# albertfgu/diffwave-sashimi

Measured on AMD Instinct MI355X. Metric: audio samples/sec (generate.py-style reverse-diffusion sampling, T=200), higher is better.
Workload: dtype f32-equivalent (3-term bf16 split, 6 products, fp32 accumulate); 1 GPU; wnet_h256_d36_T200; backbone=wavenet, batch_per_gpu=16, L=16000, T=200, parallelism=independent clips per GPU, no collective, sampler=hipGraph replay, on-device Philox noise

## Files before the change

### diffwave-sashimi_amd/csrc/common.hip

```cpp
#include "dws_common.h"
#include "model.h"

#include <mutex>

namespace dws {

static thread_local char g_err[1024] = "";

int set_error(int code, const char* fmt, ...) {
    va_list ap;
    va_start(ap, fmt);
    vsnprintf(g_err, sizeof(g_err), fmt, ap);
    va_end(ap);
    return code;
}

static std::mutex g_prof_mu;
static bool g_prof_on = false;
static std::string g_prof_substr;
static std::vector<std::pair<hipEvent_t, hipEvent_t>> g_prof_events;

bool profile_active() { return g_prof_on; }

ProfileScope::ProfileScope(const char* name, hipStream_t s) : on(false), stream(s), e0(nullptr), e1(nullptr) {
    if (!g_prof_on) return;
    if (strstr(name, g_prof_substr.c_str()) == nullptr) return;
    hipStreamCaptureStatus st = hipStreamCaptureStatusNone;
    if (hipStreamIsCapturing(s, &st) != hipSuccess || st != hipStreamCaptureStatusNone) return;
    if (hipEventCreate(&e0) != hipSuccess || hipEventCreate(&e1) != hipSuccess) return;
    on = true;
    hipEventRecord(e0, stream);
}

ProfileScope::~ProfileScope() {
    if (!on) return;
    hipEventRecord(e1, stream);
    std::lock_guard<std::mutex> lk(g_prof_mu);
    g_prof_events.emplace_back(e0, e1);
}

__global__ void multi_copy_kernel(const CopyJob* __restrict__ jobs, int parts) {
    const CopyJob j = jobs[blockIdx.x];
    for (int64_t i = (int64_t)blockIdx.y * blockDim.x + threadIdx.x; i < j.n; i += (int64_t)parts * blockDim.x) j.dst[i] = j.src[i];
}

int launch_multi_copy(const CopyJob* table_dev, int njobs, hipStream_t s) {
    const int parts = 8;
    hipLaunchKernelGGL(multi_copy_kernel, dim3((unsigned)njobs, parts), dim3(256), 0, s, table_dev, parts);
    DWS_HIP(hipGetLastError());
    return DWS_OK;
}

}
// ... 63 lines not shown
```

### diffwave-sashimi_amd/csrc/dws_common.h

```cpp
#pragma once
#include <hip/hip_runtime.h>
#include <cstdarg>
#include <cstdint>
#include <cstdio>
#include <cstring>
#include <map>
#include <string>
#include <vector>

#include "../../include/dws.h"

namespace dws {

int set_error(int code, const char* fmt, ...);

#define DWS_CHECK(cond, code, ...)                         \
    do {                                                   \
        if (!(cond)) return ::dws::set_error((code), __VA_ARGS__); \
    } while (0)

#define DWS_HIP(expr)                                                                   \
    do {                                                                                \
        hipError_t _e = (expr);                                                         \
        if (_e != hipSuccess)                                                           \
// ... 47 lines not shown
    return fmaf(-w, (p * t) * ez, fmaxf(x, 0.f));
}
__device__ __forceinline__ float dws_gelu_grad(float x) {
    float ez;
    const float cdf = dws_norm_cdf(x, ez);
    return fmaf(x * 0.39894228040143267794f, ez, cdf);
}

constexpr int DWS_MAX_DEVICES = 16;
inline int current_device_slot() {
    int d = 0;
    (void)hipGetDevice(&d);
    return ((unsigned)d < (unsigned)DWS_MAX_DEVICES) ? d : 0;
}

__device__ __forceinline__ int xcd_remap(int bid, int nwg) {
    const int NX = 8;
    int xcd = bid % NX, idx = bid / NX;
    int q = nwg / NX, r = nwg % NX;
    int base = (xcd < r) ? xcd * (q + 1) : r * (q + 1) + (xcd - r) * q;
    return base + idx;
}

}
```

### diffwave-sashimi_amd/csrc/fftconv_kernels.hip

```cpp
#include <cstdio>
#include <cstdlib>
#include <type_traits>
#include <vector>

#include "fftconv.h"

#include "fft_core.h"

namespace dws {

__device__ __forceinline__ float gelu_f(float x) { return dws_gelu(x); }
__device__ __forceinline__ int brev(int k, int bits) { return brev_bits(k, bits); }

struct NoStamp {
    __device__ __forceinline__ void operator()() const {}
    __device__ __forceinline__ void loads_landed() const {}
};
constexpr int FFT_TRACE_SLOTS = 16, FFT_TRACE_ROWS = 4;
struct WaveStamp {
    unsigned long long* slot;
    int k;
    bool lane0;
    __device__ __forceinline__ void operator()() {
        const unsigned long long t = __builtin_amdgcn_s_memtime();
// ... 669 lines not shown
    static constexpr int THREADS = M / 16;
    static constexpr size_t LDS = (size_t)(M + M / 16) * 8;
    static constexpr bool FUSED = FftPlan<LOG2M>::TAIL4 && !FftPlan<LOG2M>::ODD;
};

bool fftconv_supported(int L, int* log2m) {
    if (L < 16 || (L & 1)) return false;
    int lg = 4;
    while ((1 << lg) < L) ++lg;
    if (lg < 10) lg = 10;
    if (lg > 14) return false;
    if (log2m) *log2m = lg;
    return true;
}

static int cu_count() {
    static int n_dev[DWS_MAX_DEVICES] = {};
    int& n = n_dev[current_device_slot()];
    if (!n) {
        int dev = 0;
        hipDeviceProp_t prop;
        if (hipGetDevice(&dev) == hipSuccess && hipGetDeviceProperties(&prop, dev) == hipSuccess) n = prop.multiProcessorCount;
        if (n <= 0) n = 256;
    }
    return n;
}

template <int LOG2M>
static int fft_trace_launch(FftConvArgs a, int nwg, hipStream_t s) {
    using C = FcCfg<LOG2M>;
    static const char* names[12] = {"", "loads landed", "top pass", "fwd P1", "fwd P2", "fwd tail", "pointwise", "inv tail",
                                    "inv P2", "inv P1", "bottom + stores", "closing barrier"};
    static const bool fused = C::FUSED && getenv("DWS_FFT_NO_FUSED_TAIL") == nullptr;
    auto kern = fused ? fftconv_kernel<LOG2M, C::THREADS, true, C::FUSED> : fftconv_kernel<LOG2M, C::THREADS, true>;
    constexpr int NP = FftPlan<LOG2M>::N16 - 1;
    const int T4 = (FftPlan<LOG2M>::TAIL4 && !fused) ? 1 : 0, NST = 3 + NP + T4 + 1 + T4 + NP + 2;
    static bool attr_dev[DWS_MAX_DEVICES] = {};
    bool& attr = attr_dev[current_device_slot()];
    if (!attr) {
        DWS_HIP(hipFuncSetAttribute((const void*)kern, hipFuncAttributeMaxDynamicSharedMemorySize, (int)C::LDS));
        attr = true;
    }
// ... 223 lines not shown
```

### diffwave-sashimi_amd/csrc/wavenet.h

```cpp
#pragma once
#include "dws_common.h"

namespace dws {

constexpr int WN_LAYER_KC = 32;
constexpr int WN_BX3_KC = 16;

struct WnLayerArgs {
    const float* x_in;
    float* x_out;
    float* skip;
    const float* part_t;
    int part_t_bstride;
    const float* A1;
    const float* A2;
    const float* Abt;
    int abt_bstride;
    const int* step_idx;
    int abt_tstride, part_t_tstride;
    const float* Wd;
    const float* Wr;
    const float* Ws;
    const float* bias1;
    const float* bias2;
    const float* melc;
    int mel_bstride;
    float* gate_ws;
    float* hsave;
    int B, L, dilation, first_layer, last_layer;
    const float* wscale;
    unsigned long long* trace;
};

struct WnFinalArgs {
    const float* skip;
    const float* Af;
    const float* Wf;
    const float* bf;
    const float* Wz;
    const float* bz;
    float* out;
    float* tap;
    float scale;
    int B, L, Cout;
    int af_scaled;
// ... 17 lines not shown
int launch_wn_layer_generic(int C, int S, const WnLayerArgs& a, hipStream_t s);
bool wn_final_mfma_supported(int S);
bool wn_layer_wino_supported(int C, int S);
int launch_wino_dconv(const float* w, float* out, int C, hipStream_t s);
int launch_wn_wino_bias(const float* Wd_all, const float* part_t, float* Abt, int NL, int B, int C, hipStream_t s);
int launch_wn_layer_wino(int C, int S, const WnLayerArgs& a, hipStream_t s);
bool wn_layer_bf16x3_supported(int C, int S);
int launch_wn_layer_bf16x3(int C, int S, const WnLayerArgs& a, hipStream_t s);
int launch_pack_a_bf16x3(const float* w, void* out, int M, int K, hipStream_t s);
int launch_wn_bias_tap_bf16(const float* Wd_all, const float* part_t, const float* bias1_all, void* Abt, int NL, int B, int C,
                            hipStream_t s);
enum { WN_SPLIT_BF16X6 = 0, WN_SPLIT_F16X3 = 1 };
inline int wn_split_terms(int split) { return split == WN_SPLIT_F16X3 ? 2 : 3; }
bool wn_layer_bx6_supported(int C, int S);
int launch_wn_layer_bx6(int C, int S, const WnLayerArgs& a, int split, hipStream_t s);
int launch_weight_scale(const float* w, size_t n, const float* bias, int nb, const float* bias_b, int nb_b, float* out, hipStream_t s);
int launch_pack_a1_bx6(const float* w, void* out, int C, int split, const float* scale, hipStream_t s);
int launch_pack_a_bx6(const float* w, void* out, int M, int K, int split, const float* scale, hipStream_t s);
int launch_gemm_bx6(const float* A, const float* B, float* C, int M, int N, int K, int split, float sa, float sb, hipStream_t s);
int launch_wn_final(int S, const WnFinalArgs& a, hipStream_t s);

}
```

### diffwave-sashimi_amd/csrc/wavenet_bx6.hip

```cpp
#include <cstdlib>
#include <type_traits>

#include "bf16_split.h"
#include "wavenet.h"
#include "wn_trace.h"

namespace dws {

#ifndef BX6_PF3
#define BX6_PF3 1
#endif
#ifndef BX6_PF2
#define BX6_PF2 2
#endif
#define BX6_PF(NT) ((NT) == 2 ? BX6_PF2 : BX6_PF3)
#ifndef BX6_T_SLOTS
#define BX6_T_SLOTS 0, 2, 3, 4, 6, 7, 9
#endif

typedef float bx6_f32x4 __attribute__((ext_vector_type(4)));

#ifdef BX6_ABL_NO_NT
#define BX6_NT 0
#else
#define BX6_NT 2
#endif
__device__ __forceinline__ bx6_f32x4 bx6_load_f4(__amdgpu_buffer_rsrc_t r, int voff, int soff) {
    return __builtin_bit_cast(bx6_f32x4, __builtin_amdgcn_raw_buffer_load_b128(r, voff, soff, BX6_NT));
}
__device__ __forceinline__ void bx6_store_f4(bx6_f32x4 v, __amdgpu_buffer_rsrc_t r, int voff, int soff) {
    typedef unsigned int u4 __attribute__((ext_vector_type(4)));
    __builtin_amdgcn_raw_buffer_store_b128(__builtin_bit_cast(u4, v), r, voff, soff, BX6_NT);
// ... 112 lines not shown
    static constexpr int RAW_FLOATS = KC * 4 * NP;
    static constexpr int BOP_BYTES = (KC / 8) * 4 * NT * NP * 16;
    static constexpr int STAGE_FLOATS = 2 * RAW_FLOATS + 2 * BOP_BYTES / 4;
    static constexpr int GATE_BYTES = (C / 8) * NT * 64 * 16;
    static constexpr int MAIN_FLOATS = STAGE_FLOATS > GATE_BYTES / 4 ? STAGE_FLOATS : GATE_BYTES / 4;
    static constexpr int TR_FLOATS = 32 * 64;
    static constexpr int LDS_FLOATS = MAIN_FLOATS + WAVES * TR_FLOATS;
    static constexpr int TITEMS = (KC / 4) * NP * 2;
    static constexpr bool HALVES = WAVES == 8 && NT == 3;
    static constexpr int SW = HALVES ? WAVES / 2 : WAVES;
    static constexpr int NPIECE = KC / (2 * SW);
    static_assert(C % 32 == 0 && S % C == 0 && C % KC == 0 && KC % 16 == 0 && KC % (2 * SW) == 0 && (SW & (SW - 1)) == 0 &&
                  (!HALVES || NCB % 2 == 0) && (TITEMS % NTH == 0) && LDS_FLOATS * 4 <= 163840, "channel counts");
};

template <typename P, int C, int S, bool EXTRA>
__global__ __launch_bounds__(C * 2, (C >= 128 ? 2 : 1)) void wn_layer_bx6_kernel(WnLayerArgs a, int log2d) {
    using T = Bx6Tile<C, S, P::NT>;
    using v8 = typename P::v8;
    using v4 = typename P::v4;
    constexpr int NT = P::NT, NPR = P::NP, NA = 2 * P::NT;
    constexpr int KC = T::KC, MS = T::MS, WAVES = T::WAVES, NCB = T::NCB, NTH = T::NTH, NKB = T::NKB;
    __shared__ __attribute__((aligned(16))) float lds[T::LDS_FLOATS];
    float* const Xraw = lds;
    char* const Bop = reinterpret_cast<char*>(lds + 2 * T::RAW_FLOATS);
    char* const gt = reinterpret_cast<char*>(lds);

    const int tid = threadIdx.x;
    const int lane = tid & 63;
    const int wave = __builtin_amdgcn_readfirstlane(tid >> 6);
    const int l31 = lane & 31, lhi = lane >> 5;
    const int L = a.L, dil = 1 << log2d;
    float* const trw = lds + T::MAIN_FLOATS + wave * T::TR_FLOATS;

    const int nblk = (L + 2 * dil - 1) >> (log2d + 1);
    const int ntl = ((nblk << log2d) + 31) >> 5;
    const int tile = xcd_remap(blockIdx.x, gridDim.x);
    const int b = __builtin_amdgcn_readfirstlane(tile / ntl);
    const int tic = tile % ntl;
#ifdef WN_TILE_ORDER_LINEAR
    const int q0 = __builtin_amdgcn_readfirstlane(tic * 32);
#else
    const int q0 = __builtin_amdgcn_readfirstlane(log2d >= 6 ? ((tic % nblk) << log2d) + (tic / nblk) * 32 : tic * 32);
#endif
    const int q = q0 + l31;
    const int p = ((q >> log2d) << (log2d + 1)) + (q & (dil - 1));

    const float* __restrict__ xb = a.x_in + (size_t)b * C * L;
    unsigned long long* __restrict__ trc = a.trace ? a.trace + ((size_t)blockIdx.x * WAVES + wave) * 32 : nullptr;
    auto stamp = [&](int i) {
        if (trc) {
            const unsigned long long t = __builtin_amdgcn_s_memtime();
            if (lane == 0) trc[i] = t;
        }
    };
    stamp(0);

    const int mt1[2] = {wave, C / 32 + wave};
    int mt2[1 + MS];
    mt2[0] = wave;
#pragma unroll
    for (int m = 0; m < MS; ++m) mt2[1 + m] = C / 32 + wave * MS + m;
    float av1[2][4], ab1[2], av2[1 + MS];
    {
        const float* Abt = a.Abt + (size_t)b * a.abt_bstride + step_row_off(a.step_idx, a.abt_tstride);
#pragma unroll
        for (int m = 0; m < 2; ++m) {
            const int row = mt1[m] * 32 + l31;
#pragma unroll
            for (int j = 0; j < 4; ++j) av1[m][j] = Abt[j * 2 * C + row];
            ab1[m] = a.bias1[row];
        }
#pragma unroll
        for (int m = 0; m < 1 + MS; ++m) av2[m] = a.bias2[mt2[m] * 32 + l31];
    }
    const float ws1 = P::SCALED ? a.wscale[0] : 1.f, ws2 = P::SCALED ? a.wscale[1] : 1.f;
    const float inv1 = 1.f / (ws1 * P::SX), inv2 = 1.f / (ws2 * P::SG);

    const bool al16 = (L % 4 == 0) && ((((size_t)a.x_in | (size_t)a.x_out | (size_t)a.skip) & 15) == 0);
    const bool contig = al16 && log2d <= 4;
    const bool x4 = contig || (al16 && log2d >= 2);
    __amdgpu_buffer_rsrc_t rXall = __builtin_amdgcn_make_buffer_rsrc((void*)xb, 0, C * L * 4, 0x00020000);
    const int pbase = (q0 >> log2d) << (log2d + 1);
    const int ob = contig ? 32 + (p - pbase) - dil : l31;
    const int os = contig ? dil : 32;
    const int x0l = p - pbase, x1l = x0l + dil;
    const int gcol0 = contig ? x0l : l31, gcol1 = contig ? x1l : 32 + l31;
    int voffA, voffB;
    if (contig) {
        const int pp = pbase - 32 + 4 * (lane & 31);
        voffA = ((unsigned)pp < (unsigned)L) ? (lhi * L + pp) * 4 : 0x7ffffff0;
        voffB = 0;
    } else if (x4) {
        const int s4 = (lane >> 3) & 3, qq = q0 + 4 * (lane & 7);
        const int pp = ((qq >> log2d) << (log2d + 1)) + (qq & (dil - 1)) + (s4 - 1) * dil;
        voffA = ((unsigned)pp < (unsigned)L) ? (lhi * L + pp) * 4 : 0x7ffffff0;
        voffB = 0;
    } else {
        voffA = (p + (lhi - 1) * dil) * 4;
        voffB = (p + (lhi + 1) * dil) * 4;
    }
#ifdef BX6_ABL_NO_ROT
// ... 28 lines not shown
    auto stage_dma = [&](int cbi) {
#pragma unroll
        for (int i = 0; i < NPIECE; ++i) stage_piece(cbi, i);
    };

    constexpr int TK = T::TITEMS / NTH, T_UNITS = 7;
    struct TState {
        float d[TK][2][3];
        v4 pa[TK][NT], pb[TK][NT];
    };
    auto transform_unit = [&](int c1, int u, TState& ts) __attribute__((always_inline)) {
        const float* xs = Xraw + (c1 & 1) * T::RAW_FLOATS;
        char* bo = Bop + (c1 & 1) * T::BOP_BYTES;
#pragma unroll
        for (int k = 0; k < TK; ++k) {
            const int i = tid + NTH * k;
            const int gi = __builtin_amdgcn_readfirstlane(i >> 6);
            const int g4 = (gi * 2 + lhi) % (KC / 4);
            const int jp = __builtin_amdgcn_readfirstlane((gi * 2) / (KC / 4));
            const bool p1 = jp != 0;
            const int h = u / 3, w = u % 3;
            if (u == T_UNITS - 1) {
                char* dst = bo + ((((g4 >> 1) * 4 + 2 * jp) * NT) * 32 + l31) * 16 + (g4 & 1) * 8;
#pragma unroll
                for (int t = 0; t < NT; ++t) {
                    *reinterpret_cast<v4*>(dst + t * 512) = ts.pa[k][t];
                    *reinterpret_cast<v4*>(dst + (NT + t) * 512) = ts.pb[k][t];
                }
            } else if (w == 0) {
                const int oa = p1 ? 3 * os : 0;
#pragma unroll
                for (int e = 0; e < 2; ++e) {
// ... 172 lines not shown
        if (cb + 2 < NCB && stages(cb + 2)) stage_dma(cb + 2);
#endif
        if (cb + 1 < NCB) do_step(cb, std::integral_constant<int, 0>{}, std::true_type{});
        else do_step(cb, std::integral_constant<int, 0>{}, std::false_type{});
        do_steps_from1(cb);
        stamp(8 + 2 * cb);
#ifndef BX6_ABL_NO_DMA_WAIT
        __builtin_amdgcn_s_waitcnt(0x0F70 | NAF);
#endif
#ifndef BX6_ABL_NO_BARRIER
        __syncthreads();
#endif
        stamp(9 + 2 * cb);
    }
    stamp(2);

    const int L4 = L * 4;
    const bool first = a.first_layer, last = a.last_layer;
    __amdgpu_buffer_rsrc_t rXo = __builtin_amdgcn_make_buffer_rsrc((void*)(a.x_out + (size_t)b * C * L), 0, C * L * 4, 0x00020000);
    __amdgpu_buffer_rsrc_t rSk = __builtin_amdgcn_make_buffer_rsrc((void*)(a.skip + (size_t)b * S * L), 0, S * L * 4, 0x00020000);
    const int p0 = ((q0 >> log2d) << (log2d + 1)) + (q0 & (dil - 1));
    int voff4;
    {
        const int n4 = (lane & 15) >> 3;
        const int pos4 = (contig ? pbase + 32 * n4 : p0 + n4 * dil) + 4 * (lane & 7);
        voff4 = (pos4 < L) ? ((lane >> 4) * L + pos4) * 4 : 0x7ffffff0;
    }
    constexpr bool PRELOAD = MS == 1;
    const int voff4s = first ? 0x7ffffff0 : voff4;
    auto load_pre = [&](int m, bx6_f32x4 (&dst)[8]) {
#pragma unroll
        for (int i = 0; i < 8; ++i) {
            if (m == 0) dst[i] = *reinterpret_cast<const bx6_f32x4*>(trw + ((lane >> 4) + 4 * i) * 64 + 4 * (lane & 15));
            else dst[i] = bx6_load_f4(rSk, voff4s, ((wave * MS + (m - 1)) * 32 + 4 * i) * L4);
        }
    };
    bx6_f32x4 pre[PRELOAD ? 1 + MS : 1][8];
    if (PRELOAD && al16) {
#pragma unroll
        for (int m = 1; m < 1 + MS; ++m) load_pre(m, pre[PRELOAD ? m : 0]);
    }

    const float* melb = (EXTRA && a.melc) ? a.melc + (size_t)(a.mel_bstride ? b : 0) * 2 * C * L : nullptr;
#pragma unroll
    for (int qd = 0; qd < 4; ++qd) {
        float g0[4], g1[4];
#pragma unroll
        for (int e = 0; e < 4; ++e) {
            const int r = qd * 4 + e;
            const int ch = wave * 32 + e + 8 * qd + 4 * lhi;
#pragma unroll
            for (int n = 0; n < 2; ++n) {
                const int pos = p + n * dil;
                float ht, hs;
                if (n == 0) {
                    ht = (acc[0][0][r] + acc[0][1][r]) + acc[0][2][r];
                    hs = (acc[1][0][r] + acc[1][1][r]) + acc[1][2][r];
                } else {
                    ht = (acc[0][1][r] - acc[0][2][r]) - acc[0][3][r];
                    hs = (acc[1][1][r] - acc[1][2][r]) - acc[1][3][r];
                }
                if (P::SCALED) { ht *= inv1; hs *= inv1; }
                if (EXTRA && melb && pos < L) {
                    ht += melb[(size_t)ch * L + pos];
                    hs += melb[(size_t)(C + ch) * L + pos];
                }
                if (EXTRA && a.hsave && pos < L) {
                    float* __restrict__ hb = a.hsave + (size_t)b * 2 * C * L;
                    hb[(size_t)ch * L + pos] = ht;
                    hb[(size_t)(C + ch) * L + pos] = hs;
                }
                const float g = bx6_gate(ht, hs) * P::SG;
                if (n == 0) g0[e] = g; else g1[e] = g;
            }
        }
        v4 s0[NT], s1[NT];
        P::split4(g0, s0);
        P::split4(g1, s1);
        char* dst = gt + ((wave * 4 + qd) * NT * 64) * 16 + lhi * 8;
#pragma unroll
        for (int t = 0; t < NT; ++t) {
            *reinterpret_cast<v4*>(dst + (t * 64 + gcol0) * 16) = s0[t];
            *reinterpret_cast<v4*>(dst + (t * 64 + gcol1) * 16) = s1[t];
        }
    }
    stamp(3);

    __amdgpu_buffer_rsrc_t rA2 = __builtin_amdgcn_make_buffer_rsrc((void*)a.A2, 0, (C + S) * C * 2 * NT, 0x00020000);
    v8 c_cur[1 + MS][NT], c_nxt[1 + MS][NT];
    auto load_a2 = [&](v8 (&dst)[1 + MS][NT], int kb, int m0) {
#pragma unroll
        for (int m = m0; m < 1 + MS; ++m)
#pragma unroll
            for (int t = 0; t < NT; ++t)
                dst[m][t] = __builtin_bit_cast(v8, __builtin_amdgcn_raw_buffer_load_b128(rA2, lane16, ((mt2[m] * NKB + kb) * NT + t) * 1024, 0));
    };
    const int rot2 = rot * (KC / 16);
    auto kblock_of = [&](int kb) { const int k = kb + rot2; return k >= NKB ? k - NKB : k; };
    bx_f32x16 acc2[1 + MS][2];
    auto gemm2 = [&](auto WITH_RES) {
        constexpr int M0 = decltype(WITH_RES)::value ? 0 : 1;
        load_a2(c_cur, kblock_of(0), M0);
        {
            const v8 bf = P::bvals(lhi ? 0.f : P::SG, 0.f);
            bx_f32x16 zero;
#pragma unroll
            for (int r = 0; r < 16; ++r) zero[r] = 0.f;
#pragma unroll
            for (int m = M0; m < 1 + MS; ++m) {
                v8 af[NT];
                P::rank2(av2[m] * ws2, 0.f, lhi == 0, af);
#pragma unroll
                for (int n = 0; n < 2; ++n) {
                    acc2[m][n] = zero;
#pragma unroll
                    for (int t = NT - 1; t >= 0; --t) acc2[m][n] = P::mfma(af[t], bf, acc2[m][n]);
                }
            }
        }
        __syncthreads();
        stamp(4);
        const char* gb = gt + lhi * (NT * 64 * 16) + l31 * 16;
#pragma unroll 2
        for (int kb = 0; kb < NKB; ++kb) {
            const int kbn = (kb + 1 < NKB) ? kb + 1 : kb;
            load_a2(c_nxt, kblock_of(kbn), M0);
            __builtin_amdgcn_sched_barrier(0);
            const char* gk = gb + kblock_of(kb) * (2 * NT * 64 * 16);
            v8 bq[2][NT];
#pragma unroll
            for (int n = 0; n < 2; ++n)
#pragma unroll
                for (int t = 0; t < NT; ++t) bq[n][t] = *reinterpret_cast<const v8*>(gk + (t * 64 + n * 32) * 16);
#pragma unroll
            for (int t = 0; t < NPR; ++t)
#pragma unroll
                for (int m = M0; m < 1 + MS; ++m)
// ... 8 lines not shown
    };
    if (last) gemm2(std::false_type{});
    else gemm2(std::true_type{});
    stamp(5);

    const float rs = 0.70710678118654752440f;
    if (al16) {
#pragma unroll
        for (int m = 0; m < 1 + MS; ++m) {
            if (m == 0 && last) continue;
            if (!PRELOAD || m == 0) load_pre(m, pre[0]);
            asm volatile("s_waitcnt lgkmcnt(0)" ::: "memory");
#pragma unroll
            for (int n = 0; n < 2; ++n)
#pragma unroll
                for (int r = 0; r < 16; ++r) trw[((r & 3) + 8 * (r >> 2) + 4 * lhi) * 64 + n * 32 + l31] = P::SCALED ? acc2[m][n][r] * inv2 : acc2[m][n][r];
            asm volatile("s_waitcnt lgkmcnt(0)" ::: "memory");
            const int row0 = (m == 0) ? wave * 32 : (wave * MS + (m - 1)) * 32;
#pragma unroll
            for (int i = 0; i < 8; ++i) {
                const bx6_f32x4 v = *reinterpret_cast<const bx6_f32x4*>(trw + ((lane >> 4) + 4 * i) * 64 + 4 * (lane & 15));
                bx6_f32x4 o = pre[PRELOAD ? m : 0][i] + v;
                if (m == 0) o = o * rs;
                bx6_store_f4(o, m == 0 ? rXo : rSk, voff4, (row0 + 4 * i) * L4);
                asm volatile("s_nop 1" ::: "memory");
            }
            asm volatile("" ::: "memory");
        }
    } else {
        int voffn[2];
#pragma unroll
        for (int n = 0; n < 2; ++n) {
            const int pos = contig ? pbase + 32 * n + l31 : p + n * dil;
            voffn[n] = (pos < L) ? (4 * lhi * L + pos) * 4 : 0x7ffffff0;
        }
#pragma unroll
        for (int n = 0; n < 2; ++n) {
            if (!last) {
                const int s0 = (wave * 32) * L4;
#pragma unroll
                for (int r = 0; r < 16; ++r) {
                    const int so = s0 + ((r & 3) + 8 * (r >> 2)) * L4;
                    const float x = __builtin_bit_cast(float, __builtin_amdgcn_raw_buffer_load_b32(rXall, voffn[n], so, 0));
                    const float v = (x + (P::SCALED ? acc2[0][n][r] * inv2 : acc2[0][n][r])) * rs;
                    __builtin_amdgcn_raw_buffer_store_b32(__builtin_bit_cast(unsigned, v), rXo, voffn[n], so, 0);
                }
            }
#pragma unroll
            for (int m = 0; m < MS; ++m) {
                const int s0 = ((wave * MS + m) * 32) * L4;
#pragma unroll
                for (int r = 0; r < 16; ++r) {
                    const int so = s0 + ((r & 3) + 8 * (r >> 2)) * L4;
                    const float old = first ? 0.f : __builtin_bit_cast(float, __builtin_amdgcn_raw_buffer_load_b32(rSk, voffn[n], so, 0));
                    const float v = old + (P::SCALED ? acc2[1 + m][n][r] * inv2 : acc2[1 + m][n][r]);
                    __builtin_amdgcn_raw_buffer_store_b32(__builtin_bit_cast(unsigned, v), rSk, voffn[n], so, 0);
                }
            }
        }
    }
    stamp(6);
    if (trc) {
        __builtin_amdgcn_s_waitcnt(0);
        stamp(7);
    }
}

template <typename P, int C, int S>
static int launch_bx6_t(const WnLayerArgs& a, int log2d, hipStream_t s) {
    ProfileScope ps(P::NT == 3 ? "wn_layer_bx6" : "wn_layer_f16x3", s);
    using T = Bx6Tile<C, S, P::NT>;
    const int dil = 1 << log2d;
    const int nblk = (a.L + 2 * dil - 1) / (2 * dil);
    const int ntl = (nblk * dil + 31) / 32;
    const int ntiles = a.B * ntl;
    static const bool trace = std::getenv("DWS_BX6_TRACE") != nullptr;
    if (trace && !a.melc && !a.hsave) {
        wino_trace_launch(ntiles, T::WAVES, a, s, [&](const WnLayerArgs& at) {
            hipLaunchKernelGGL((wn_layer_bx6_kernel<P, C, S, false>), dim3(ntiles), dim3(T::NTH), 0, s, at, log2d);
        }, P::NT == 3 ? "bx6" : "f16x3");
        return DWS_OK;
    }
    if (a.melc || a.hsave) hipLaunchKernelGGL((wn_layer_bx6_kernel<P, C, S, true>), dim3(ntiles), dim3(T::NTH), 0, s, a, log2d);
    else hipLaunchKernelGGL((wn_layer_bx6_kernel<P, C, S, false>), dim3(ntiles), dim3(T::NTH), 0, s, a, log2d);
    return DWS_OK;
}

bool wn_layer_bx6_supported(int C, int S) {
    return (C == 64 && S == 64) || (C == 128 && S == 128) || (C == 128 && S == 256) || (C == 256 && S == 256);
}

template <typename P>
static int launch_bx6_p(int C, int S, const WnLayerArgs& a, int log2d, hipStream_t s) {
    if (C == 64 && S == 64) return launch_bx6_t<P, 64, 64>(a, log2d, s);
    if (C == 128 && S == 128) return launch_bx6_t<P, 128, 128>(a, log2d, s);
    if (C == 128 && S == 256) return launch_bx6_t<P, 128, 256>(a, log2d, s);
    if (C == 256 && S == 256) return launch_bx6_t<P, 256, 256>(a, log2d, s);
    return set_error(DWS_ERR_UNSUPPORTED, "wn_layer_bx6: (C=%d,S=%d) not instantiated", C, S);
}

// ... 70 lines not shown
```

### diffwave-sashimi_amd/csrc/wavenet_model.hip

```cpp
#include <cmath>

#include "conditioner.h"
#include "model.h"
#include "wavenet.h"
#include "wavenet_backward.h"

namespace dws {

struct WaveNetModel : dws_model {
    int Cin, Cout, C, S, NL, cycle, Ein, Emid, Eout, MB;
    bool cond, mfma_layer, mfma_final;
    bool bf16x3 = false;
    bool bf16x6 = false;
    bool f16x3 = false;
    DevBuf wscale;
    bool wino_opt = true;
    bool wino_fits(int64_t nL) const {
        return (int64_t)std::max(C, S) * nL * 4 < ((int64_t)1 << 31) && nL + 4 * ((int64_t)1 << (cycle - 1)) < ((int64_t)1 << 28);
    }
    bool wino() const { return wino_opt && mfma_layer && !bf16x3 && !bf16x6 && !f16x3 && wn_layer_wino_supported(C, S) && (L == 0 || wino_fits(L)); }
    bool wino_rows() const { return wino() || bf16x6 || f16x3; }

    DevBuf Wi;
    std::vector<DevBuf> A1, Wrs, A2, bias2;
// ... 11 lines not shown
    DevBuf mel_u0, mel_u1;
    int64_t melBm = 0;
    DevBuf mel_in;
    int mel_T = 0;
    CondTrainWs cws;
    DevBuf gW0f, gW1f, gWcf;
    DevBuf x0, x1, skip, gate, emb, h1, h2, part_t, scratch_out;
    std::vector<DevBuf> tx, tH;
    std::vector<DevBuf> ATd, ATg;
    std::vector<DevBuf> ATw;
    DevBuf ATf, wpart, bpart;
    bool mfma_bwd = false;
    uint64_t commit_version = 0, bwd_pack_version = ~0ull;
    DevBuf ty, ta1, ta2, dxa, dxb, dskip, dgb, dHb, dresb, dyb, dWfold, dpt, dh2, dh1, demb, dWt_all, dbt_all;
    bool trained_fwd = false;

    explicit WaveNetModel(const dws_model_desc& dd) {
        d = dd;
        Cin = d.in_channels; Cout = d.out_channels; C = d.res_channels; S = d.skip_channels;
        NL = d.num_res_layers; cycle = d.dilation_cycle;
        Ein = d.diffusion_step_embed_dim_in; Emid = d.diffusion_step_embed_dim_mid; Eout = d.diffusion_step_embed_dim_out;
        MB = d.mel_bands;
        cond = !d.unconditional;
        mfma_layer = wn_layer_mfma_supported(C, S);
        mfma_bwd = tapconv_mfma_supported(C, S, C, 1) && tapconv_mfma_supported(C, 2 * C, 0, 3) &&
                   tapconv_mfma_supported(S, S, 0, 1) && std::getenv("DWS_WAVENET_GENERIC_BWD") == nullptr;
        mfma_final = wn_final_mfma_supported(S);
        if (std::getenv("DWS_WN_DIRECT")) wino_opt = false;
        auto wn = [&](const std::string& p, std::vector<int64_t> vshape) {
            std::vector<int64_t> g(vshape.size(), 1);
// ... 46 lines not shown
                          "precision=bf16x6 is not built for (res_channels=%d, skip_channels=%d)", C, S);
                bf16x6 = true; bf16x3 = f16x3 = false; dirty = true; trained_fwd = false;
                return DWS_OK;
            }
            if (value == "f16x3") {
                DWS_CHECK(mfma_layer && wn_layer_bx6_supported(C, S), DWS_ERR_UNSUPPORTED,
                          "precision=f16x3 is not built for (res_channels=%d, skip_channels=%d)", C, S);
                f16x3 = true; bf16x3 = bf16x6 = false; dirty = true; trained_fwd = false;
                return DWS_OK;
            }
        }
        if (key == "conv_algo") {
            if (value == "winograd") { wino_opt = true; dirty = true; trained_fwd = false; return DWS_OK; }
            if (value == "direct") { wino_opt = false; dirty = true; trained_fwd = false; return DWS_OK; }
        }
        return dws_model::set_option(key, value);
    }

    float* Wd(int n) const { return Wd_all.f() + (size_t)n * 2 * C * C * 3; }

    int fold(const std::string& p, float* out, int O, int inner, hipStream_t s) {
        return launch_fold_weight_norm(P(p + ".weight_v"), P(p + ".weight_g"), out, O, inner, s);
    }

    int commit(hipStream_t s) override {
        DWS_TRY(Wi.ensure((size_t)C * Cin * 4));
        DWS_TRY(fold("init_conv.0.conv", Wi.f(), C, Cin, s));
        DWS_TRY(Wt_all.ensure((size_t)NL * C * Eout * 4));
        DWS_TRY(bt_all.ensure((size_t)NL * C * 4));
        DWS_TRY(b1_all.ensure((size_t)NL * 2 * C * 4));
        DWS_TRY(Wd_all.ensure((size_t)NL * 2 * C * C * 3 * 4));
        if (mfma_layer) DWS_TRY(tmp_pack.ensure((size_t)2 * C * 4 * C * 4));
        stack_params.begin();
        for (int n = 0; n < NL; ++n) {
            const std::string p = "residual_layer.residual_blocks." + std::to_string(n);
            stack_params.add(P(p + ".fc_t.weight"), Wt_all.f() + (size_t)n * C * Eout, (size_t)C * Eout);
            stack_params.add(P(p + ".fc_t.bias"), bt_all.f() + (size_t)n * C, (size_t)C);
            stack_params.add(P(p + ".dilated_conv_layer.conv.bias"), b1_all.f() + (size_t)n * 2 * C, (size_t)2 * C);
            DWS_TRY(fold(p + ".dilated_conv_layer.conv", Wd(n), 2 * C, C * 3, s));
            DWS_TRY(Wrs[n].ensure((size_t)(C + S) * C * 4));
// ... 280 lines not shown
                a.Abt = mfma_layer ? tab_abt.f() + (size_t)n * tab_T * arow : nullptr; a.abt_bstride = 0; a.abt_tstride = arow;
                a.step_idx = step_idx;
            } else {
                a.part_t = part_t.f() + (size_t)n * C; a.part_t_bstride = NL * C;
                a.Abt = mfma_layer ? Abt.f() + (size_t)n * B * arow : nullptr; a.abt_bstride = arow;
            }
            a.Wd = Wd(n); a.Wr = Wrs[n].f(); a.Ws = Wrs[n].f() + (size_t)C * C;
            a.bias1 = P(p + ".dilated_conv_layer.conv.bias");
            a.bias2 = bias2[n].f();
            a.melc = melBm ? melc.f() + (size_t)n * melBm * 2 * C * L : nullptr;
            a.mel_bstride = (melBm > 1) ? 1 : 0;
            a.gate_ws = gate.f();
            a.B = (int)B; a.L = (int)L;
            a.dilation = 1 << (n % cycle);
            a.first_layer = (n == 0); a.last_layer = (n == NL - 1);
            if (mfma_layer && bf16x3) DWS_TRY(launch_wn_layer_bf16x3(C, S, a, s));
            else if (bf16x6) DWS_TRY(launch_wn_layer_bx6(C, S, a, WN_SPLIT_BF16X6, s));
            else if (f16x3) { a.wscale = wscale.f() + 2 * n; DWS_TRY(launch_wn_layer_bx6(C, S, a, WN_SPLIT_F16X3, s)); }
            else if (wino()) DWS_TRY(launch_wn_layer_wino(C, S, a, s));
            else if (mfma_layer) DWS_TRY(launch_wn_layer_mfma(C, S, a, s));
            else DWS_TRY(launch_wn_layer_generic(C, S, a, s));
        }
        DWS_TRY(final_stage(out, train ? ty.f() : nullptr, s));
        DWS_HIP(hipGetLastError());
        return DWS_OK;
    }

    int wn_bwd(const std::string& p, const float* dWf, int O, int inner, hipStream_t s) {
        return launch_weight_norm_bwd(dWf, P(p + ".weight_v"), P(p + ".weight_g"), G(p + ".weight_v"), G(p + ".weight_g"), O,
                                      inner, s);
// ... 190 lines not shown
```

### diffwave-sashimi_amd/csrc/wn_trace.h

```cpp
#pragma once
#include <cstdio>
#include <cstdlib>
#include <vector>

#include "wavenet.h"

namespace dws {

template <typename F>
static void wino_trace_launch(int nwg, int waves, WnLayerArgs a, hipStream_t s, F launch, const char* tag = "wino") {
    unsigned long long* d = nullptr;
    const size_t n = (size_t)nwg * waves * 32;
    if (hipMalloc(&d, n * 8) != hipSuccess) return;
    (void)hipMemsetAsync(d, 0, n * 8, s);
    a.trace = d;
    launch(a);
    (void)hipStreamSynchronize(s);
    std::vector<unsigned long long> h(n);
    (void)hipMemcpy(h.data(), d, n * 8, hipMemcpyDeviceToHost);
    (void)hipFree(d);
    double ph[8] = {0};
    static double chunk[8][32];
    for (auto& c : chunk) for (double& v : c) v = 0;
    double g2[8] = {0}, ep[8] = {0};
    double wgspan = 0;
// ... 3 lines not shown
            const unsigned long long* t = &h[((size_t)g * waves + w) * 32];
            for (int i = 1; i < 8; ++i) ph[i] += (double)(t[i] - t[i - 1]);
            if (w < 8) { g2[w] += (double)(t[5] - t[4]); ep[w] += (double)(t[6] - t[5]); }
            if (w < 8)
                for (int i = 8; i < 32; ++i)
                    if (t[i]) { chunk[w][i] += (double)(t[i] - t[1]); }
            if (t[0] < g0) g0 = t[0];
            if (t[7] > g1) g1 = t[7];
        }
        wgspan += (double)(g1 - g0);
    }
    const double nw = (double)nwg * waves;
    fprintf(stderr, "[%s trace] d=%d wgs=%d per-wave mean cycles: prologue %.0f gemm1 %.0f "
            "extra+gate %.0f barrier %.0f gemm2 %.0f epilogue %.0f drain %.0f; mean workgroup span %.0f\n", tag, a.dilation, nwg, ph[1] / nw, ph[2] / nw, ph[3] / nw, ph[4] / nw, ph[5] / nw,
            ph[6] / nw, ph[7] / nw, wgspan / nwg);
    if (std::getenv("DWS_WINO_TRACE_CHUNKS")) {
        fprintf(stderr, "  per-wave gemm2 / epilogue ticks:");
        for (int w = 0; w < waves && w < 8; ++w) fprintf(stderr, " %.0f/%.0f", g2[w] / nwg, ep[w] / nwg);
        fprintf(stderr, "\n");
    }
    if (std::getenv("DWS_WINO_TRACE_CHUNKS"))
        for (int w = 0; w < waves && w < 8; ++w) {
            fprintf(stderr, "  wave %d arrive/release since gemm1 start:", w);
            for (int i = 8; i < 24; ++i) fprintf(stderr, " %.0f%s", chunk[w][i] / nwg, (i & 1) ? " |" : "");
            fprintf(stderr, "\n");
        }
}

}
```

Baseline: 33730 audio samples/s.

## Make bx6 WaveNet layer kernel persistent with a resident-sized grid

The bx6 layer kernel body becomes a device tile function. The kernel now loops over tiles with a grid stride, and for C=256 it launches by default only as many workgroups as can be resident (CU count times occupancy), instead of one workgroup per tile. Kernel arguments are re-read from the kernarg segment and lane/wave ids are recomputed, apparently to cut register pressure across the loop. The aim is to remove the workgroup launch/tail cost and the imbalance from the extra waves. In exchange, each tile adds a waitcnt plus a barrier, and tiles inside one workgroup no longer overlap.

After: 33770 audio samples/s (median of 2 runs). No clear change (+0.1%).

```diff
diff --git a/diffwave-sashimi_amd/csrc/common.hip b/diffwave-sashimi_amd/csrc/common.hip
--- a/diffwave-sashimi_amd/csrc/common.hip
+++ b/diffwave-sashimi_amd/csrc/common.hip
@@ -37,6 +37,18 @@
     hipEventRecord(e1, stream);
     std::lock_guard<std::mutex> lk(g_prof_mu);
     g_prof_events.emplace_back(e0, e1);
+}
+
+int cu_count() {
+    static int n_dev[DWS_MAX_DEVICES] = {};
+    int& n = n_dev[current_device_slot()];
+    if (!n) {
+        int dev = 0;
+        hipDeviceProp_t prop;
+        if (hipGetDevice(&dev) == hipSuccess && hipGetDeviceProperties(&prop, dev) == hipSuccess) n = prop.multiProcessorCount;
+        if (n <= 0) n = 256;
+    }
+    return n;
 }
 
 __global__ void multi_copy_kernel(const CopyJob* __restrict__ jobs, int parts) {
diff --git a/diffwave-sashimi_amd/csrc/dws_common.h b/diffwave-sashimi_amd/csrc/dws_common.h
--- a/diffwave-sashimi_amd/csrc/dws_common.h
+++ b/diffwave-sashimi_amd/csrc/dws_common.h
@@ -85,6 +85,8 @@
     return ((unsigned)d < (unsigned)DWS_MAX_DEVICES) ? d : 0;
 }
 
+int cu_count();
+
 __device__ __forceinline__ int xcd_remap(int bid, int nwg) {
     const int NX = 8;
     int xcd = bid % NX, idx = bid / NX;
diff --git a/diffwave-sashimi_amd/csrc/fftconv_kernels.hip b/diffwave-sashimi_amd/csrc/fftconv_kernels.hip
--- a/diffwave-sashimi_amd/csrc/fftconv_kernels.hip
+++ b/diffwave-sashimi_amd/csrc/fftconv_kernels.hip
@@ -707,18 +707,6 @@
     return true;
 }
 
-static int cu_count() {
-    static int n_dev[DWS_MAX_DEVICES] = {};
-    int& n = n_dev[current_device_slot()];
-    if (!n) {
-        int dev = 0;
-        hipDeviceProp_t prop;
-        if (hipGetDevice(&dev) == hipSuccess && hipGetDeviceProperties(&prop, dev) == hipSuccess) n = prop.multiProcessorCount;
-        if (n <= 0) n = 256;
-    }
-    return n;
-}
-
 template <int LOG2M>
 static int fft_trace_launch(FftConvArgs a, int nwg, hipStream_t s) {
     using C = FcCfg<LOG2M>;
diff --git a/diffwave-sashimi_amd/csrc/wavenet.h b/diffwave-sashimi_amd/csrc/wavenet.h
--- a/diffwave-sashimi_amd/csrc/wavenet.h
+++ b/diffwave-sashimi_amd/csrc/wavenet.h
@@ -29,6 +29,7 @@
     float* hsave;
     int B, L, dilation, first_layer, last_layer;
     const float* wscale;
+    int bx6_grid;
     unsigned long long* trace;
 };
 
@@ -76,6 +77,7 @@
 inline int wn_split_terms(int split) { return split == WN_SPLIT_F16X3 ? 2 : 3; }
 bool wn_layer_bx6_supported(int C, int S);
 int launch_wn_layer_bx6(int C, int S, const WnLayerArgs& a, int split, hipStream_t s);
+void wn_layer_bx6_warm(int C, int S);
 int launch_weight_scale(const float* w, size_t n, const float* bias, int nb, const float* bias_b, int nb_b, float* out, hipStream_t s);
 int launch_pack_a1_bx6(const float* w, void* out, int C, int split, const float* scale, hipStream_t s);
 int launch_pack_a_bx6(const float* w, void* out, int M, int K, int split, const float* scale, hipStream_t s);
diff --git a/diffwave-sashimi_amd/csrc/wavenet_bx6.hip b/diffwave-sashimi_amd/csrc/wavenet_bx6.hip
--- a/diffwave-sashimi_amd/csrc/wavenet_bx6.hip
+++ b/diffwave-sashimi_amd/csrc/wavenet_bx6.hip
@@ -1,4 +1,5 @@
 #include <cstdlib>
+#include <cstring>
 #include <type_traits>
 
 #include "bf16_split.h"
@@ -16,6 +17,10 @@
 #define BX6_PF(NT) ((NT) == 2 ? BX6_PF2 : BX6_PF3)
 #ifndef BX6_T_SLOTS
 #define BX6_T_SLOTS 0, 2, 3, 4, 6, 7, 9
+#endif
+
+#ifndef BX6_AUTO_PERSISTENT
+#define BX6_AUTO_PERSISTENT(C, NT) ((C) == 256)
 #endif
 
 typedef float bx6_f32x4 __attribute__((ext_vector_type(4)));
@@ -158,8 +163,19 @@
                   (!HALVES || NCB % 2 == 0) && (TITEMS % NTH == 0) && LDS_FLOATS * 4 <= 163840, "channel counts");
 };
 
+__device__ __forceinline__ WnLayerArgs bx6_kargs() {
+    WnLayerArgs r;
+    typedef const __attribute__((address_space(4))) unsigned long long* KargWords;
+    KargWords p = (KargWords)__builtin_amdgcn_kernarg_segment_ptr();
+    asm volatile("" : "+s"(p));
+    static_assert(alignof(WnLayerArgs) == 8 && sizeof(WnLayerArgs) % 8 == 0, "copied as 8-byte words");
+    __builtin_memcpy(&r, p, sizeof(r));
+    return r;
+}
+
 template <typename P, int C, int S, bool EXTRA>
-__global__ __launch_bounds__(C * 2, (C >= 128 ? 2 : 1)) void wn_layer_bx6_kernel(WnLayerArgs a, int log2d) {
+__device__ __forceinline__ void bx6_tile(const int log2d, const int vb, const int ntiles, const int wave0) {
+    const WnLayerArgs a = bx6_kargs();
     using T = Bx6Tile<C, S, P::NT>;
     using v8 = typename P::v8;
     using v4 = typename P::v4;
@@ -170,16 +186,17 @@
     char* const Bop = reinterpret_cast<char*>(lds + 2 * T::RAW_FLOATS);
     char* const gt = reinterpret_cast<char*>(lds);
 
-    const int tid = threadIdx.x;
-    const int lane = tid & 63;
-    const int wave = __builtin_amdgcn_readfirstlane(tid >> 6);
+    int lane, wave = wave0;
+    asm volatile("v_mbcnt_lo_u32_b32 %0, -1, 0\n\tv_mbcnt_hi_u32_b32 %0, -1, %0" : "=v"(lane));
+    asm volatile("" : "+s"(wave));
+    wave = __builtin_amdgcn_readfirstlane(wave);
     const int l31 = lane & 31, lhi = lane >> 5;
     const int L = a.L, dil = 1 << log2d;
     float* const trw = lds + T::MAIN_FLOATS + wave * T::TR_FLOATS;
 
     const int nblk = (L + 2 * dil - 1) >> (log2d + 1);
     const int ntl = ((nblk << log2d) + 31) >> 5;
-    const int tile = xcd_remap(blockIdx.x, gridDim.x);
+    const int tile = xcd_remap(vb, ntiles);
     const int b = __builtin_amdgcn_readfirstlane(tile / ntl);
     const int tic = tile % ntl;
 #ifdef WN_TILE_ORDER_LINEAR
@@ -191,10 +208,11 @@
     const int p = ((q >> log2d) << (log2d + 1)) + (q & (dil - 1));
 
     const float* __restrict__ xb = a.x_in + (size_t)b * C * L;
-    unsigned long long* __restrict__ trc = a.trace ? a.trace + ((size_t)blockIdx.x * WAVES + wave) * 32 : nullptr;
+    const int tracing = __builtin_amdgcn_readfirstlane(a.trace != nullptr);
     auto stamp = [&](int i) {
-        if (trc) {
+        if (tracing) {
             const unsigned long long t = __builtin_amdgcn_s_memtime();
+            unsigned long long* trc = bx6_kargs().trace + ((size_t)vb * WAVES + wave) * 32;
             if (lane == 0) trc[i] = t;
         }
     };
@@ -205,7 +223,7 @@
     mt2[0] = wave;
 #pragma unroll
     for (int m = 0; m < MS; ++m) mt2[1 + m] = C / 32 + wave * MS + m;
-    float av1[2][4], ab1[2], av2[1 + MS];
+    float av1[2][4], ab1[2];
     {
         const float* Abt = a.Abt + (size_t)b * a.abt_bstride + step_row_off(a.step_idx, a.abt_tstride);
 #pragma unroll
@@ -215,8 +233,6 @@
             for (int j = 0; j < 4; ++j) av1[m][j] = Abt[j * 2 * C + row];
             ab1[m] = a.bias1[row];
         }
-#pragma unroll
-        for (int m = 0; m < 1 + MS; ++m) av2[m] = a.bias2[mt2[m] * 32 + l31];
     }
     const float ws1 = P::SCALED ? a.wscale[0] : 1.f, ws2 = P::SCALED ? a.wscale[1] : 1.f;
     const float inv1 = 1.f / (ws1 * P::SX), inv2 = 1.f / (ws2 * P::SG);
@@ -228,8 +244,6 @@
     const int pbase = (q0 >> log2d) << (log2d + 1);
     const int ob = contig ? 32 + (p - pbase) - dil : l31;
     const int os = contig ? dil : 32;
-    const int x0l = p - pbase, x1l = x0l + dil;
-    const int gcol0 = contig ? x0l : l31, gcol1 = contig ? x1l : 32 + l31;
     int voffA, voffB;
     if (contig) {
         const int pp = pbase - 32 + 4 * (lane & 31);
@@ -288,8 +302,7 @@
         char* bo = Bop + (c1 & 1) * T::BOP_BYTES;
 #pragma unroll
         for (int k = 0; k < TK; ++k) {
-            const int i = tid + NTH * k;
-            const int gi = __builtin_amdgcn_readfirstlane(i >> 6);
+            const int gi = wave + WAVES * k;
             const int g4 = (gi * 2 + lhi) % (KC / 4);
             const int jp = __builtin_amdgcn_readfirstlane((gi * 2) / (KC / 4));
             const bool p1 = jp != 0;
@@ -492,24 +505,35 @@
         stamp(9 + 2 * cb);
     }
     stamp(2);
+    const WnLayerArgs al = bx6_kargs();
+    int lane_g = lane;
+    asm volatile("" : "+v"(lane_g));
+    const int l31g = lane_g & 31, lhig = lane_g >> 5;
+    const int qg = q0 + l31g;
+    const int pg = ((qg >> log2d) << (log2d + 1)) + (qg & (dil - 1));
+    const int x0l = pg - pbase, x1l = x0l + dil;
+    const int gcol0 = contig ? x0l : l31g, gcol1 = contig ? x1l : 32 + l31g;
+    float av2[1 + MS];
+#pragma unroll
+    for (int m = 0; m < 1 + MS; ++m) av2[m] = al.bias2[mt2[m] * 32 + l31g];
 
     const int L4 = L * 4;
-    const bool first = a.first_layer, last = a.last_layer;
-    __amdgpu_buffer_rsrc_t rXo = __builtin_amdgcn_make_buffer_rsrc((void*)(a.x_out + (size_t)b * C * L), 0, C * L * 4, 0x00020000);
-    __amdgpu_buffer_rsrc_t rSk = __builtin_amdgcn_make_buffer_rsrc((void*)(a.skip + (size_t)b * S * L), 0, S * L * 4, 0x00020000);
+    const bool first = al.first_layer, last = al.last_layer;
+    __amdgpu_buffer_rsrc_t rXo = __builtin_amdgcn_make_buffer_rsrc((void*)(al.x_out + (size_t)b * C * L), 0, C * L * 4, 0x00020000);
+    __amdgpu_buffer_rsrc_t rSk = __builtin_amdgcn_make_buffer_rsrc((void*)(al.skip + (size_t)b * S * L), 0, S * L * 4, 0x00020000);
     const int p0 = ((q0 >> log2d) << (log2d + 1)) + (q0 & (dil - 1));
     int voff4;
     {
-        const int n4 = (lane & 15) >> 3;
-        const int pos4 = (contig ? pbase + 32 * n4 : p0 + n4 * dil) + 4 * (lane & 7);
-        voff4 = (pos4 < L) ? ((lane >> 4) * L + pos4) * 4 : 0x7ffffff0;
+        const int n4 = (lane_g & 15) >> 3;
+        const int pos4 = (contig ? pbase + 32 * n4 : p0 + n4 * dil) + 4 * (lane_g & 7);
+        voff4 = (pos4 < L) ? ((lane_g >> 4) * L + pos4) * 4 : 0x7ffffff0;
     }
     constexpr bool PRELOAD = MS == 1;
     const int voff4s = first ? 0x7ffffff0 : voff4;
     auto load_pre = [&](int m, bx6_f32x4 (&dst)[8]) {
 #pragma unroll
         for (int i = 0; i < 8; ++i) {
-            if (m == 0) dst[i] = *reinterpret_cast<const bx6_f32x4*>(trw + ((lane >> 4) + 4 * i) * 64 + 4 * (lane & 15));
+            if (m == 0) dst[i] = *reinterpret_cast<const bx6_f32x4*>(trw + ((lane_g >> 4) + 4 * i) * 64 + 4 * (lane_g & 15));
             else dst[i] = bx6_load_f4(rSk, voff4s, ((wave * MS + (m - 1)) * 32 + 4 * i) * L4);
         }
     };
@@ -519,17 +543,17 @@
         for (int m = 1; m < 1 + MS; ++m) load_pre(m, pre[PRELOAD ? m : 0]);
     }
 
-    const float* melb = (EXTRA && a.melc) ? a.melc + (size_t)(a.mel_bstride ? b : 0) * 2 * C * L : nullptr;
+    const float* melb = (EXTRA && al.melc) ? al.melc + (size_t)(al.mel_bstride ? b : 0) * 2 * C * L : nullptr;
 #pragma unroll
     for (int qd = 0; qd < 4; ++qd) {
         float g0[4], g1[4];
 #pragma unroll
         for (int e = 0; e < 4; ++e) {
             const int r = qd * 4 + e;
-            const int ch = wave * 32 + e + 8 * qd + 4 * lhi;
+            const int ch = wave * 32 + e + 8 * qd + 4 * lhig;
 #pragma unroll
             for (int n = 0; n < 2; ++n) {
-                const int pos = p + n * dil;
+                const int pos = pg + n * dil;
                 float ht, hs;
                 if (n == 0) {
                     ht = (acc[0][0][r] + acc[0][1][r]) + acc[0][2][r];
@@ -543,8 +567,8 @@
                     ht += melb[(size_t)ch * L + pos];
                     hs += melb[(size_t)(C + ch) * L + pos];
                 }
-                if (EXTRA && a.hsave && pos < L) {
-                    float* __restrict__ hb = a.hsave + (size_t)b * 2 * C * L;
+                if (EXTRA && al.hsave && pos < L) {
+                    float* __restrict__ hb = al.hsave + (size_t)b * 2 * C * L;
                     hb[(size_t)ch * L + pos] = ht;
                     hb[(size_t)(C + ch) * L + pos] = hs;
                 }
@@ -555,7 +579,7 @@
         v4 s0[NT], s1[NT];
         P::split4(g0, s0);
         P::split4(g1, s1);
-        char* dst = gt + ((wave * 4 + qd) * NT * 64) * 16 + lhi * 8;
+        char* dst = gt + ((wave * 4 + qd) * NT * 64) * 16 + lhig * 8;
 #pragma unroll
         for (int t = 0; t < NT; ++t) {
             *reinterpret_cast<v4*>(dst + (t * 64 + gcol0) * 16) = s0[t];
@@ -564,7 +588,7 @@
     }
     stamp(3);
 
-    __amdgpu_buffer_rsrc_t rA2 = __builtin_amdgcn_make_buffer_rsrc((void*)a.A2, 0, (C + S) * C * 2 * NT, 0x00020000);
+    __amdgpu_buffer_rsrc_t rA2 = __builtin_amdgcn_make_buffer_rsrc((void*)al.A2, 0, (C + S) * C * 2 * NT, 0x00020000);
     v8 c_cur[1 + MS][NT], c_nxt[1 + MS][NT];
     auto load_a2 = [&](v8 (&dst)[1 + MS][NT], int kb, int m0) {
 #pragma unroll
@@ -580,14 +604,14 @@
         constexpr int M0 = decltype(WITH_RES)::value ? 0 : 1;
         load_a2(c_cur, kblock_of(0), M0);
         {
-            const v8 bf = P::bvals(lhi ? 0.f : P::SG, 0.f);
+            const v8 bf = P::bvals(lhig ? 0.f : P::SG, 0.f);
             bx_f32x16 zero;
 #pragma unroll
             for (int r = 0; r < 16; ++r) zero[r] = 0.f;
 #pragma unroll
             for (int m = M0; m < 1 + MS; ++m) {
                 v8 af[NT];
-                P::rank2(av2[m] * ws2, 0.f, lhi == 0, af);
+                P::rank2(av2[m] * ws2, 0.f, lhig == 0, af);
 #pragma unroll
                 for (int n = 0; n < 2; ++n) {
                     acc2[m][n] = zero;
@@ -598,7 +622,7 @@
         }
         __syncthreads();
         stamp(4);
-        const char* gb = gt + lhi * (NT * 64 * 16) + l31 * 16;
+        const char* gb = gt + lhig * (NT * 64 * 16) + l31g * 16;
 #pragma unroll 2
         for (int kb = 0; kb < NKB; ++kb) {
             const int kbn = (kb + 1 < NKB) ? kb + 1 : kb;
@@ -637,12 +661,12 @@
 #pragma unroll
             for (int n = 0; n < 2; ++n)
 #pragma unroll
-                for (int r = 0; r < 16; ++r) trw[((r & 3) + 8 * (r >> 2) + 4 * lhi) * 64 + n * 32 + l31] = P::SCALED ? acc2[m][n][r] * inv2 : acc2[m][n][r];
+                for (int r = 0; r < 16; ++r) trw[((r & 3) + 8 * (r >> 2) + 4 * lhig) * 64 + n * 32 + l31g] = P::SCALED ? acc2[m][n][r] * inv2 : acc2[m][n][r];
             asm volatile("s_waitcnt lgkmcnt(0)" ::: "memory");
             const int row0 = (m == 0) ? wave * 32 : (wave * MS + (m - 1)) * 32;
 #pragma unroll
             for (int i = 0; i < 8; ++i) {
-                const bx6_f32x4 v = *reinterpret_cast<const bx6_f32x4*>(trw + ((lane >> 4) + 4 * i) * 64 + 4 * (lane & 15));
+                const bx6_f32x4 v = *reinterpret_cast<const bx6_f32x4*>(trw + ((lane_g >> 4) + 4 * i) * 64 + 4 * (lane_g & 15));
                 bx6_f32x4 o = pre[PRELOAD ? m : 0][i] + v;
                 if (m == 0) o = o * rs;
                 bx6_store_f4(o, m == 0 ? rXo : rSk, voff4, (row0 + 4 * i) * L4);
@@ -654,8 +678,8 @@
         int voffn[2];
 #pragma unroll
         for (int n = 0; n < 2; ++n) {
-            const int pos = contig ? pbase + 32 * n + l31 : p + n * dil;
-            voffn[n] = (pos < L) ? (4 * lhi * L + pos) * 4 : 0x7ffffff0;
+            const int pos = contig ? pbase + 32 * n + l31g : pg + n * dil;
+            voffn[n] = (pos < L) ? (4 * lhig * L + pos) * 4 : 0x7ffffff0;
         }
 #pragma unroll
         for (int n = 0; n < 2; ++n) {
@@ -683,10 +707,46 @@
         }
     }
     stamp(6);
-    if (trc) {
+    if (tracing) {
         __builtin_amdgcn_s_waitcnt(0);
         stamp(7);
     }
+}
+
+template <typename P, int C, int S, bool EXTRA>
+__global__ __launch_bounds__(C * 2, (C >= 128 ? 2 : 1)) void wn_layer_bx6_kernel(WnLayerArgs a, int log2d, int ntiles) {
+    const int G = gridDim.x;
+    const int wave0 = __builtin_amdgcn_readfirstlane(threadIdx.x >> 6);
+    for (int v = blockIdx.x; v < ntiles; v += G) {
+        bx6_tile<P, C, S, EXTRA>(log2d, v, ntiles, wave0);
+        if (v + G < ntiles) {
+            __builtin_amdgcn_s_waitcnt(0);
+            __syncthreads();
+        }
+    }
+}
+
+template <typename P, int C, int S, bool EXTRA>
+static int bx6_resident_grid() {
+    static int g_dev[DWS_MAX_DEVICES] = {};
+    int& g = g_dev[current_device_slot()];
+    if (!g) {
+        int r = 0;
+        if (hipOccupancyMaxActiveBlocksPerMultiprocessor(&r, wn_layer_bx6_kernel<P, C, S, EXTRA>, Bx6Tile<C, S, P::NT>::NTH, 0) != hipSuccess || r < 1) r = 1;
+        g = cu_count() * r;
+    }
+    return g;
+}
+
+static int bx6_env_grid() {
+    static const int v = [] {
+        const char* e = std::getenv("DWS_BX6_GRID");
+        if (!e || !*e || !std::strcmp(e, "auto")) return 0;
+        if (!std::strcmp(e, "tiles")) return -1;
+        const int n = std::atoi(e);
+        return n >= 1 ? n : 0;
+    }();
+    return v;
 }
 
 template <typename P, int C, int S>
@@ -697,16 +757,37 @@
     const int nblk = (a.L + 2 * dil - 1) / (2 * dil);
     const int ntl = (nblk * dil + 31) / 32;
     const int ntiles = a.B * ntl;
+    const bool extra = a.melc || a.hsave;
+    const int want = a.bx6_grid ? a.bx6_grid : bx6_env_grid();
+    int grid = ntiles;
+    if (want > 0) grid = want < ntiles ? want : ntiles;
+    else if (want == 0 && BX6_AUTO_PERSISTENT(C, P::NT)) {
+        const int g = extra ? bx6_resident_grid<P, C, S, true>() : bx6_resident_grid<P, C, S, false>();
+        grid = g < ntiles ? g : ntiles;
+    }
     static const bool trace = std::getenv("DWS_BX6_TRACE") != nullptr;
-    if (trace && !a.melc && !a.hsave) {
+    if (trace && !extra) {
         wino_trace_launch(ntiles, T::WAVES, a, s, [&](const WnLayerArgs& at) {
-            hipLaunchKernelGGL((wn_layer_bx6_kernel<P, C, S, false>), dim3(ntiles), dim3(T::NTH), 0, s, at, log2d);
-        }, P::NT == 3 ? "bx6" : "f16x3");
+            hipLaunchKernelGGL((wn_layer_bx6_kernel<P, C, S, false>), dim3(grid), dim3(T::NTH), 0, s, at, log2d, ntiles);
+        }, P::NT == 3 ? "bx6" : "f16x3", grid);
         return DWS_OK;
     }
-    if (a.melc || a.hsave) hipLaunchKernelGGL((wn_layer_bx6_kernel<P, C, S, true>), dim3(ntiles), dim3(T::NTH), 0, s, a, log2d);
-    else hipLaunchKernelGGL((wn_layer_bx6_kernel<P, C, S, false>), dim3(ntiles), dim3(T::NTH), 0, s, a, log2d);
+    if (extra) hipLaunchKernelGGL((wn_layer_bx6_kernel<P, C, S, true>), dim3(grid), dim3(T::NTH), 0, s, a, log2d, ntiles);
+    else hipLaunchKernelGGL((wn_layer_bx6_kernel<P, C, S, false>), dim3(grid), dim3(T::NTH), 0, s, a, log2d, ntiles);
     return DWS_OK;
+}
+
+template <typename P, int C, int S>
+static void bx6_warm_t() {
+    (void)bx6_resident_grid<P, C, S, false>();
+    (void)bx6_resident_grid<P, C, S, true>();
+}
+
+void wn_layer_bx6_warm(int C, int S) {
+    if (C == 64 && S == 64) { bx6_warm_t<SplitBf16x3, 64, 64>(); bx6_warm_t<SplitF16x2, 64, 64>(); }
+    if (C == 128 && S == 128) { bx6_warm_t<SplitBf16x3, 128, 128>(); bx6_warm_t<SplitF16x2, 128, 128>(); }
+    if (C == 128 && S == 256) { bx6_warm_t<SplitBf16x3, 128, 256>(); bx6_warm_t<SplitF16x2, 128, 256>(); }
+    if (C == 256 && S == 256) { bx6_warm_t<SplitBf16x3, 256, 256>(); bx6_warm_t<SplitF16x2, 256, 256>(); }
 }
 
 bool wn_layer_bx6_supported(int C, int S) {
diff --git a/diffwave-sashimi_amd/csrc/wavenet_model.hip b/diffwave-sashimi_amd/csrc/wavenet_model.hip
--- a/diffwave-sashimi_amd/csrc/wavenet_model.hip
+++ b/diffwave-sashimi_amd/csrc/wavenet_model.hip
@@ -49,6 +49,7 @@
     uint64_t commit_version = 0, bwd_pack_version = ~0ull;
     DevBuf ty, ta1, ta2, dxa, dxb, dskip, dgb, dHb, dresb, dyb, dWfold, dpt, dh2, dh1, demb, dWt_all, dbt_all;
     bool trained_fwd = false;
+    int bx6_grid = 0;
 
     explicit WaveNetModel(const dws_model_desc& dd) {
         d = dd;
@@ -125,6 +126,16 @@
             if (value == "winograd") { wino_opt = true; dirty = true; trained_fwd = false; return DWS_OK; }
             if (value == "direct") { wino_opt = false; dirty = true; trained_fwd = false; return DWS_OK; }
         }
+        if (key == "bx6_grid") {
+            char* end = nullptr;
+            const long n = std::strtol(value.c_str(), &end, 10);
+            if (value == "auto") bx6_grid = 0;
+            else if (value == "tiles") bx6_grid = -1;
+            else if (end != value.c_str() && *end == 0 && n >= 1 && n <= (1 << 30)) bx6_grid = (int)n;
+            else return set_error(DWS_ERR_INVALID, "bx6_grid=%s: auto, tiles or a workgroup count >= 1", value.c_str());
+            dirty = true;
+            return DWS_OK;
+        }
         return dws_model::set_option(key, value);
     }
 
@@ -135,6 +146,7 @@
     }
 
     int commit(hipStream_t s) override {
+        if (bf16x6 || f16x3) wn_layer_bx6_warm(C, S);
         DWS_TRY(Wi.ensure((size_t)C * Cin * 4));
         DWS_TRY(fold("init_conv.0.conv", Wi.f(), C, Cin, s));
         DWS_TRY(Wt_all.ensure((size_t)NL * C * Eout * 4));
@@ -445,6 +457,7 @@
             a.B = (int)B; a.L = (int)L;
             a.dilation = 1 << (n % cycle);
             a.first_layer = (n == 0); a.last_layer = (n == NL - 1);
+            a.bx6_grid = bx6_grid;
             if (mfma_layer && bf16x3) DWS_TRY(launch_wn_layer_bf16x3(C, S, a, s));
             else if (bf16x6) DWS_TRY(launch_wn_layer_bx6(C, S, a, WN_SPLIT_BF16X6, s));
             else if (f16x3) { a.wscale = wscale.f() + 2 * n; DWS_TRY(launch_wn_layer_bx6(C, S, a, WN_SPLIT_F16X3, s)); }
diff --git a/diffwave-sashimi_amd/csrc/wn_trace.h b/diffwave-sashimi_amd/csrc/wn_trace.h
--- a/diffwave-sashimi_amd/csrc/wn_trace.h
+++ b/diffwave-sashimi_amd/csrc/wn_trace.h
@@ -8,7 +8,7 @@
 namespace dws {
 
 template <typename F>
-static void wino_trace_launch(int nwg, int waves, WnLayerArgs a, hipStream_t s, F launch, const char* tag = "wino") {
+static void wino_trace_launch(int nwg, int waves, WnLayerArgs a, hipStream_t s, F launch, const char* tag = "wino", int grid = 0) {
     unsigned long long* d = nullptr;
     const size_t n = (size_t)nwg * waves * 32;
     if (hipMalloc(&d, n * 8) != hipSuccess) return;
@@ -42,6 +42,23 @@
     fprintf(stderr, "[%s trace] d=%d wgs=%d per-wave mean cycles: prologue %.0f gemm1 %.0f "
             "extra+gate %.0f barrier %.0f gemm2 %.0f epilogue %.0f drain %.0f; mean workgroup span %.0f\n", tag, a.dilation, nwg, ph[1] / nw, ph[2] / nw, ph[3] / nw, ph[4] / nw, ph[5] / nw,
             ph[6] / nw, ph[7] / nw, wgspan / nwg);
+    if (grid > 0 && grid < nwg) {
+        double gap = 0, wgap = 0;
+        for (int g = 0; g + grid < nwg; ++g) {
+            unsigned long long e1 = 0, b0 = ~0ull;
+            for (int w = 0; w < waves; ++w) {
+                const unsigned long long* t = &h[((size_t)g * waves + w) * 32];
+                const unsigned long long* u = &h[((size_t)(g + grid) * waves + w) * 32];
+                if (t[7] > e1) e1 = t[7];
+                if (u[0] < b0) b0 = u[0];
+                wgap += (double)(long long)(u[0] - t[7]);
+            }
+            gap += (double)(long long)(b0 - e1);
+        }
+        const double np = (double)(nwg - grid);
+        fprintf(stderr, "  between tiles (grid %d, %d tiles): last stamp of a tile -> first stamp of the workgroup's next tile %.0f cycles; "
+                "per wave %.0f\n", grid, nwg, gap / np, wgap / (np * waves));
+    }
     if (std::getenv("DWS_WINO_TRACE_CHUNKS")) {
         fprintf(stderr, "  per-wave gemm2 / epilogue ticks:");
         for (int w = 0; w < waves && w < 8; ++w) fprintf(stderr, " %.0f/%.0f", g2[w] / nwg, ep[w] / nwg);
```
